# tp7/Sushi

Measured on NVIDIA H100. Metric: subtitle_events_per_s, higher is better.
Workload: dtype f32

## Files before the change

sushi_b200/csrc/sb_fused2.cu:

```cuda
#include "sb_internal.h"
#include <cmath>
#include <cstdlib>
#include <vector>

#include "sb_fused_common.cuh"
#include "sb_fft_smem.cuh"

using namespace sb;
using namespace sbf;

#ifndef SB_V2_SPECIAL_PREFETCH
#define SB_V2_SPECIAL_PREFETCH 1
#endif

namespace {

constexpr int QB = 16384;
constexpr int QT = 512;
constexpr int QNW = QT / 32;
constexpr int Q4 = QB / 4;
constexpr int QBLK = 256;
constexpr int QROW = kQuadRowF2 / 2;
__host__ __device__ constexpr int qa(int i) { return i < Q4 ? (i >> 8) * (2 * QBLK) + (i & (QBLK - 1)) : 2 * Q4; }
__host__ __device__ constexpr int qm(int i) { return i < Q4 ? qa(i) + QBLK : 2 * Q4 + 1; }
static_assert(QROW >= 2 * Q4 + 2 && (QROW * 16) % 128 == 0, "row layout");
constexpr int kDA = 529, kDB = 33;
constexpr int QPHYS = 16 * kDA;
constexpr int kUU = kDA;

struct PackedTables {
    const float2* wb;
    const float4* d1;
    const float4* d2;
};

__device__ constexpr float kC64[8] = {1.0f, 0.99518472667219689f, 0.98078528040323043f, 0.95694033573220882f,
                                      0.92387953251128674f, 0.88192126434835503f, 0.83146961230254524f, 0.77301045336273696f};
__device__ constexpr float kS64[8] = {0.0f, 0.098017140329560602f, 0.19509032201612825f, 0.29028467725446233f,
                                      0.38268343236508978f, 0.47139673682599764f, 0.55557023301960218f, 0.63439328416364549f};

struct C2 { float2 r, i; };
template <bool V> struct BoolTag { static constexpr bool value = V; };

__device__ __forceinline__ float2 neg2(float2 a) { return make_float2(-a.x, -a.y); }
__device__ __forceinline__ float2 add2(float2 a, float2 b) { return make_float2(__fadd_rn(a.x, b.x), __fadd_rn(a.y, b.y)); }
__device__ __forceinline__ float2 sub2(float2 a, float2 b) { return add2(a, neg2(b)); }
__device__ __forceinline__ float2 mul2(float2 a, float2 b) { return make_float2(__fmul_rn(a.x, b.x), __fmul_rn(a.y, b.y)); }
__device__ __forceinline__ float2 fma2(float2 a, float2 b, float2 c) { return make_float2(__fmaf_rn(a.x, b.x, c.x), __fmaf_rn(a.y, b.y, c.y)); }
__device__ __forceinline__ float2 bc(float s) { return make_float2(s, s); }

__device__ __forceinline__ C2 cadd2(C2 a, C2 b) { return {add2(a.r, b.r), add2(a.i, b.i)}; }
__device__ __forceinline__ C2 csub2(C2 a, C2 b) { return {sub2(a.r, b.r), sub2(a.i, b.i)}; }
__device__ __forceinline__ C2 cmul_s(C2 a, float c, float s) {
    C2 o;
    o.r = fma2(a.r, bc(c), mul2(a.i, bc(-s)));
    o.i = fma2(a.r, bc(s), mul2(a.i, bc(c)));
    return o;
}
__device__ __forceinline__ C2 from4(float4 v) { return {make_float2(v.x, v.y), make_float2(v.z, v.w)}; }

__device__ __forceinline__ C2 rot32p(C2 d, int q) {
    if (q == 0) return d;
    if (q == 8) return {neg2(d.i), d.r};
    const float h = 0.70710678118654752f;
    if (q == 4) return {mul2(sub2(d.r, d.i), bc(h)), mul2(add2(d.r, d.i), bc(h))};
    if (q == 12) return {mul2(add2(d.r, d.i), bc(-h)), mul2(sub2(d.r, d.i), bc(h))};
    return cmul_s(d, kC32[q], kS32[q]);
}

template <int HI = 8, int LO = 1>
__device__ __forceinline__ void dft16p(C2 (&v)[16]) {
#pragma unroll
    for (int h = HI; h >= LO; h >>= 1) {
#pragma unroll
        for (int g = 0; g < 16; g += 2 * h) {
#pragma unroll
            for (int a = 0; a < h; ++a) {
                const C2 x = v[g + a], y = v[g + a + h];
                v[g + a] = cadd2(x, y);
                v[g + a + h] = rot32p(csub2(x, y), a * (16 / h));
            }
        }
    }
}

__device__ __forceinline__ constexpr int phys(int n) { return (n >> 9) * kDA + ((n >> 5) & 15) * kDB + (n & 31); }
struct Buf {
    float2* r; float2* i;
    __device__ __forceinline__ C2 ld(int p) const { return {r[p], i[p]}; }
    __device__ __forceinline__ void st(int p, C2 v) const { r[p] = v.r; i[p] = v.i; }
};

struct Rows {
    static constexpr int STRIDE = QROW;
    static __device__ __forceinline__ int unit(int tid, int uu) { return (tid >> 8) * (2 * QBLK) + (tid & (QBLK - 1)) + uu * (2 * QT); }
    static constexpr int USTEP = 2 * QT;
    static __device__ __forceinline__ void load(const float4* row, int u, float4& a, float4& m) { a = __ldg(row + u); m = __ldg(row + u + QBLK); }
    static __device__ __forceinline__ void loadp(const float4* row, int u, bool pred, float4& a, float4& m) {
        const float4 zero4 = make_float4(0.f, 0.f, 0.f, 0.f);
        a = pred ? __ldg(row + u) : zero4;  m = pred ? __ldg(row + u + QBLK) : zero4;
    }
    static __device__ __forceinline__ void load_special(const float4* row, float4& a, float4& m) { a = __ldg(row + qa(Q4)); m = __ldg(row + qm(Q4)); }
};

__device__ __forceinline__ void pack_quad(float2 aR, float2 aI, float2 mR, float2 mI, float c, float s,
                                          C2& lo, C2& hi) {
    const float2 eR = add2(aR, mR), eI = sub2(aI, mI);
    const float2 dR = sub2(aR, mR), dI = add2(aI, mI);
    const float2 wR = make_float2(c, -s), wI = make_float2(s, c);
    const float2 oR = fma2(dR, wR, neg2(mul2(dI, wI)));
    const float2 oI = fma2(dR, wI, mul2(dI, wR));
    const float2 zloR = sub2(eR, oI), zloI = add2(eI, oR);
    const float2 zhiR = add2(eR, oI), zhiI = sub2(oR, eI);
    const float c2 = fmaf(c, c, -s * s), s2 = 2.0f * c * s;
    {
        const float ur = zloR.x + zloR.y, ui = zloI.x + zloI.y;
        const float dr = zloR.x - zloR.y, di = zloI.x - zloI.y;
        lo.r = make_float2(ur, dr * c2 - di * s2);  lo.i = make_float2(ui, dr * s2 + di * c2);
    }
    {
        const float ur = zhiR.y + zhiR.x, ui = zhiI.y + zhiI.x;
        const float dr = zhiR.y - zhiR.x, di = zhiI.y - zhiI.x;
        hi.r = make_float2(ur, -(dr * c2) - di * s2);  hi.i = make_float2(ui, dr * s2 - di * c2);
    }
}

constexpr int kRounds = QB / (QT * 8);
constexpr int kLagsPerRound = QT * 8;

struct Smem {
    Buf buf;
    double2* base;
    unsigned char* lo;
    unsigned char* hi;
    unsigned char* end;
    __device__ __forceinline__ explicit Smem(unsigned char* raw) {
        buf.r = reinterpret_cast<float2*>(raw); buf.i = buf.r + QPHYS;
        base = reinterpret_cast<double2*>(raw + (size_t)QPHYS * 16);
        lo = reinterpret_cast<unsigned char*>(base + kRounds * QNW * 2);
        hi = lo + QB + 16;
        end = hi + QB + 48;
    }
};
constexpr int kSmallBytes = 512;
constexpr size_t kSmemCommon = (size_t)QPHYS * 16 + kRounds * QNW * 2 * sizeof(double2) + (QB + 16) + (QB + 48);

struct Item {
    QueryDesc d; int q; int64_t k, j_blk;
    __device__ __forceinline__ Item(const QueryDesc& dd, int qq, int64_t kk) : d(dd), q(qq), k(kk), j_blk(kk * QB) {}
    __device__ __forceinline__ Item(const QueryDesc* desc, const int* item_query, int64_t item_first, int64_t local) {
        q = __ldg(item_query + local);
        d = desc[q];
        k = d.k0 + (item_first + local - d.itemBase);
        j_blk = k * QB;
    }
};

template <bool WARP_BASES = false>
__device__ __forceinline__ void stage_inputs(const Item& it, int tid, const uint8_t* img8, int64_t img_n,
                                             const double2* ipfx, const Smem& sm, unsigned long long* bar) {
    const int64_t hi0 = (it.j_blk + it.d.tlen) & ~(int64_t)15;
    const int64_t limit = (img_n + 16) & ~(int64_t)15;
    if (tid == 0) {
        int64_t lo_bytes = limit - it.j_blk; if (lo_bytes > QB + 16) lo_bytes = QB + 16; if (lo_bytes < 0) lo_bytes = 0;
        int64_t hi_bytes = limit - hi0;      if (hi_bytes > QB + 48) hi_bytes = QB + 48; if (hi_bytes < 0) hi_bytes = 0;
// ... 379 lines not shown
        const float f_w0q = (float)(Wq + 0.25 + (double)oq);
        const float f_A = (float)(Cw + (double)(oq - bi2 * os));
        float cc[8];
#pragma unroll
        for (int e = 0; e < 2; ++e) {
            const C2 E = buf.ld(ech + kDA * (2 * r + e)), O = buf.ld(ech + kDA * (2 * r + e) + 1);
            const float2 xr = fma2(O.r, bc(wc), fma2(O.i, bc(-ws), E.r));
            const float2 xi = fma2(O.r, bc(ws), fma2(O.i, bc(wc), E.i));
            cc[4 * e + 0] = xr.x; cc[4 * e + 1] = xi.x; cc[4 * e + 2] = xr.y; cc[4 * e + 3] = xi.y;
        }
        const float cmax = fmaxf(fmaxf(fmaxf(cc[0], cc[1]), fmaxf(cc[2], cc[3])), fmaxf(fmaxf(cc[4], cc[5]), fmaxf(cc[6], cc[7])));
        const int64_t j0 = jt + 8 * r;
        const bool some = interior || (j0 < jhi && j0 + 8 > jlo);
        const bool inside = interior || (j0 >= jlo && j0 + 8 <= jhi);
        const float lbn = fmaf(cmax, m2s, f_A - f_delta), ubn = lbn + 2.0f * f_delta;
        const float lbv = lbn * rsqrt_fast(f_w0q + kRunQ) * 0.999999f;
        run_lb[r] = !some ? kSent : (lbn >= 0.f ? lbv : -kSent);
        const float ubv = ubn * rsqrt_fast(f_w0q - kRunQ) * 1.000001f;
        if (inside && f_w0q > 4.0f * kRunQ && ubn >= 0.f) tmin = fminf(tmin, ubv);
        oq += tq[r]; os += ts[r];
    }
#pragma unroll
    for (int o = 16; o > 0; o >>= 1) tmin = fminf(tmin, __shfl_xor_sync(0xffffffffu, tmin, o));
    if (lane == 0) s_min[warp] = tmin;
    fence_proxy_async();
    csync<ID>();
    static_assert(NW == 16, "block minimum over 16 warps");
    float bmin = s_min[lane & (NW - 1)];
#pragma unroll
    for (int o = NW / 2; o > 0; o >>= 1) bmin = fminf(bmin, __shfl_xor_sync(0xffffffffu, bmin, o));
    const float thr = bmin + m_rt;
    const bool all = curve_out != nullptr || !(bmin < sat);
    unsigned left = 0;
#pragma unroll
    for (int r = 0; r < RUNS; ++r) left |= (run_lb[r] <= thr || (all && run_lb[r] < kSent)) ? (1u << r) : 0u;
    if (left && sink.recs != nullptr && !all) {
#pragma unroll 1
        for (int r = 0; r < RUNS; ++r) {
            if (!((left >> r) & 1u)) continue;
            const int slot = atomicAdd(sink.s_cnt, 1);
            if (slot >= kRunSlots) break;
            float cc[8];
            const int k3 = warp;
#pragma unroll
            for (int e = 0; e < 2; ++e) {
                const C2 E = buf.ld(ech + kDA * (2 * r + e)), O = buf.ld(ech + kDA * (2 * r + e) + 1);
                const float2 w = make_float2(kC32[k3], kS32[k3]);
                const float2 xr = fma2(O.r, bc(w.x), fma2(O.i, bc(-w.y), E.r));
                const float2 xi = fma2(O.r, bc(w.y), fma2(O.i, bc(w.x), E.i));
                cc[4 * e + 0] = xr.x; cc[4 * e + 1] = xi.x; cc[4 * e + 2] = xr.y; cc[4 * e + 3] = xi.y;
            }
            float4* r4 = reinterpret_cast<float4*>(sink.recs + slot);
            const int64_t j0 = jt + 8 * r;
            *reinterpret_cast<int4*>(r4) = make_int4(it.q, 1, (int)(unsigned)(j0 & 0xffffffffll), (int)(j0 >> 32));
            r4[1] = make_float4(cc[0], cc[1], cc[2], cc[3]);
            r4[2] = make_float4(cc[4], cc[5], cc[6], cc[7]);
            left &= ~(1u << r);
        }
    }
    unsigned long long best = ~0ull;
    if (__any_sync(0xffffffffu, left != 0u)) {
        unsigned cand = 0;
#pragma unroll 1
        for (int r = 0; r < RUNS; ++r) {
            const bool sel = (left >> r) & 1u;
            if (!__any_sync(0xffffffffu, sel)) continue;
            const int64_t j0 = jt + 8 * r;
            float cc[8];
#pragma unroll
            for (int e = 0; e < 2; ++e) {
                const C2 E = buf.ld(ech + kDA * (2 * r + e)), O = buf.ld(ech + kDA * (2 * r + e) + 1);
                const float2 xr = fma2(O.r, bc(wc), fma2(O.i, bc(-ws), E.r));
                const float2 xi = fma2(O.r, bc(ws), fma2(O.i, bc(wc), E.i));
                cc[4 * e + 0] = xr.x; cc[4 * e + 1] = xi.x; cc[4 * e + 2] = xr.y; cc[4 * e + 3] = xi.y;
            }
            const unsigned long long lo8 = *reinterpret_cast<const unsigned long long*>(sm.lo + 32 * tid + 8 * r);
            const int hb = (int)((j_blk + n) & 15) + 32 * tid + 8 * r;
            const unsigned long long h0 = *reinterpret_cast<const unsigned long long*>(sm.hi + (hb & ~7));
            const unsigned long long h1 = *reinterpret_cast<const unsigned long long*>(sm.hi + (hb & ~7) + 8);
            const unsigned shb = (unsigned)(hb & 7) * 8u;
            const unsigned long long hi8 = shb ? ((h0 >> shb) | (h1 << (64u - shb))) : h0;
            const int2 off = s_w0[r * QT + tid];
            const float f_w0q = (float)(Wq + 0.25 + (double)off.y);
            const float f_A = (float)(Cw + (double)(off.y - bi2 * off.x));
            float v8[8];
            float vmin = kSent;
            int rq = 0, rs = 0;
#pragma unroll
            for (int i = 0; i < 8; ++i) {
                const float frq = (float)rq;
                const float num = fmaf(cc[i], m2s, fmaf(m2b, (float)rs, f_A + frq));
                const float v = num * rsqrt_fast(f_w0q + frq);
                const bool valid = sel && j0 + i >= jlo && j0 + i < jhi;
                v8[i] = valid ? v : kSent;
                vmin = fminf(vmin, v8[i]);
                const int lo = (int)((lo8 >> (8 * i)) & 0xffu), hi = (int)((hi8 >> (8 * i)) & 0xffu);
                const int dd = hi - lo;
                rq += (hi + lo) * dd; rs += dd;
            }
#pragma unroll
            for (int o = 16; o > 0; o >>= 1) vmin = fminf(vmin, __shfl_xor_sync(0xffffffffu, vmin, o));
            const float thrw = fminf(thr, vmin + m_rt);
#pragma unroll
            for (int i = 0; i < 8; ++i) cand |= (v8[i] < kSent && (v8[i] <= thrw || all)) ? (1u << (r * 8 + i)) : 0u;
        }
        while (cand) {
            const int bit = __ffs((int)cand) - 1;
            cand &= cand - 1;
            const int r = bit >> 3, i = bit & 7;
            const int m = 32 * tid + bit;
            const int64_t j = j_blk + m;
            const int jj = m >> 2;
            const int ca = (jj & 15) * kDA + ((jj >> 4) & 15) * kDB + 2 * (jj >> 8);
            const C2 E = buf.ld(ca), O = buf.ld(ca + 1);
            const float2 w = make_float2(kC32[jj >> 8], kS32[jj >> 8]);
            const bool second = (m & 2) != 0;
            const float er = second ? E.r.y : E.r.x, ei = second ? E.i.y : E.i.x, orr = second ? O.r.y : O.r.x, oi = second ? O.i.y : O.i.x;
            const float xr = fmaf(orr, w.x, fmaf(oi, -w.y, er)), xi = fmaf(orr, w.y, fmaf(oi, w.x, ei));
            const double cc = (double)((m & 1) ? xi : xr) * scale;
            const unsigned long long lo8 = *reinterpret_cast<const unsigned long long*>(sm.lo + 32 * tid + 8 * r);
            const int hb = (int)((j_blk + n) & 15) + 32 * tid + 8 * r;
            const unsigned long long h0 = *reinterpret_cast<const unsigned long long*>(sm.hi + (hb & ~7));
            const unsigned long long h1 = *reinterpret_cast<const unsigned long long*>(sm.hi + (hb & ~7) + 8);
            const unsigned shb = (unsigned)(hb & 7) * 8u;
            const unsigned long long hi8 = shb ? ((h0 >> shb) | (h1 << (64u - shb))) : h0;
            const unsigned long long keep = i ? (~0ull >> (8 * (8 - i))) : 0ull;
            const unsigned la = (unsigned)(lo8 & keep), lb = (unsigned)((lo8 & keep) >> 32), ha = (unsigned)(hi8 & keep), hb2 = (unsigned)((hi8 & keep) >> 32);
            const int rq = (int)__dp4a(ha, ha, __dp4a(hb2, hb2, 0u)) - (int)__dp4a(la, la, __dp4a(lb, lb, 0u));
            const int rs = (int)__dp4a(ha, 0x01010101u, __dp4a(hb2, 0x01010101u, 0u)) - (int)__dp4a(la, 0x01010101u, __dp4a(lb, 0x01010101u, 0u));
            const int2 off = s_w0[r * QT + tid];
            const double wsum = (Ws + (double)off.x) + (double)rs, wsq = (Wq + (double)off.y) + (double)rq;
            const float v = sqdiff_exact(cc, wsum, wsq, a, b, tsum, tsq, n_ab);
            if (curve_out) curve_out[d.curveOff + (j - jlo)] = v;
            const unsigned long long key = ((unsigned long long)__float_as_uint(v) << 32) | (unsigned int)(j - jlo);
            best = key < best ? key : best;
        }
        if (best != ~0ull) atomicMin(keys + it.q, best);
    }
    fence_proxy_async();
    csync<ID>();
    after_read();
}

template <typename S> struct QueryStreams { const float4* Xhat; int64_t nblk; const S* img; int64_t img_n; const double2* ipfx; const double2* tpfx; };
template <typename S>
__device__ __forceinline__ QueryStreams<S> select_streams(const StreamEntry* streams, const int2* slots, int q) {
    const int2 sl = slots[q];
    const StreamEntry si = streams[sl.x];
    return {reinterpret_cast<const float4*>(si.specq), si.nblk, static_cast<const S*>(si.raw), si.n, si.pfx, streams[sl.y].pfx};
}
#define SB_SELECT_STREAMS(q) do { const QueryStreams<S> qs__ = select_streams<S>(streams, slots, (q)); \
    Xhat = qs__.Xhat; nblk = qs__.nblk; img = qs__.img; img_n = qs__.img_n; ipfx = qs__.ipfx; tpfx = qs__.tpfx; } while (0)

template <typename S, int EPI, bool MULTI = false>
__global__ void __launch_bounds__(QT, 1)
k_match_packed(const float4* __restrict__ That, int64_t part_first,
               const float4* __restrict__ Xhat, int64_t nblk,
               const S* __restrict__ img, int64_t img_n,
               const double2* __restrict__ ipfx, const double2* __restrict__ tpfx,
               const QueryDesc* __restrict__ desc, const int* __restrict__ item_query, int64_t item_first,
               PackedTables tab, unsigned long long* __restrict__ keys, float* __restrict__ curve_out,
               RunRecord* __restrict__ recs, int* __restrict__ rec_count,
               const StreamEntry* __restrict__ streams = nullptr, const int2* __restrict__ slots = nullptr) {
    constexpr int T = QT, NW = QNW;
    constexpr bool is_u8 = sizeof(S) == 1;
    extern __shared__ __align__(16) unsigned char smem_raw[];
    const Smem sm(smem_raw);
    unsigned long long* s_bar = reinterpret_cast<unsigned long long*>(sm.end);
    unsigned long long* s_best = s_bar + 1;
    float* s_min = reinterpret_cast<float*>(s_best + NW);
    int* s_cnt = reinterpret_cast<int*>(sm.end + kRunCountOff());
    const RunSink sink = {EPI == 3 && recs ? recs + (size_t)blockIdx.x * kRunSlots : nullptr, s_cnt};
    float4* s_sp = reinterpret_cast<float4*>(sm.end + kSmallBytes);
    int2* s_w0 = EPI >= 2 && is_u8 ? reinterpret_cast<int2*>(sm.end + kSmallBytes + kSpecialBytes) : nullptr;
    const Buf& buf = sm.buf;

    const int tid = threadIdx.x, lane = tid & 31, warp = tid >> 5;
    const Item it(desc, item_query, item_first, blockIdx.x);
    const QueryDesc& d = it.d;
    if constexpr (MULTI) SB_SELECT_STREAMS(it.q);

    if (is_u8) {
        if (tid == 0) mbar_init(s_bar, 1);
        stage_inputs<EPI == 3>(it, tid, reinterpret_cast<const uint8_t*>(img), img_n, ipfx, sm, s_bar);
    }
    if (EPI == 3 && tid == 96) *s_cnt = 0;
    if (EPI >= 2 && tid == 64) query_constants<S>(reinterpret_cast<double2*>(sm.end + kQueryConstOff()), d, img_n, ipfx, tpfx);

    {
        int P = d.P;
        if (it.k + P > nblk) P = (int)(nblk - it.k);
        typedef Rows R;
        const float4* tp = That + (d.partBase - part_first) * (int64_t)R::STRIDE;
        const float4* xp = Xhat + it.k * (int64_t)R::STRIDE;
        const float2 wbase = __ldg(tab.wb + tid);
        const int tm = (T - tid) & (T - 1);
        const int col = phys(tid), mcol = phys(tm);
        const bool sp_pref = EPI >= 2 && SB_V2_SPECIAL_PREFETCH && special_fits(d.P, 1);
        if (sp_pref && warp == NW - 1) special_prefetch(s_sp, tp, xp, d.P, 1, it.k, nblk, lane);
        constexpr int U = 4;
#pragma unroll 1
        for (int half = 0; half < 2; ++half) {
            const int i0 = R::unit(tid, half * U);
            QuadAcc acc[U];
#pragma unroll
            for (int u = 0; u < U; ++u) acc[u].zero();
#pragma unroll 1
            for (int p = 0; p < P; ++p) {
                const float4* t = tp + (int64_t)p * R::STRIDE;
                const float4* x = xp + (int64_t)p * R::STRIDE;
                float4 ta[U], tmm[U], xa[U], xm[U];
#pragma unroll
                for (int u = 0; u < U; ++u) {
                    R::load(t, i0 + u * R::USTEP, ta[u], tmm[u]);
                    R::load(x, i0 + u * R::USTEP, xa[u], xm[u]);
                }
#pragma unroll
                for (int u = 0; u < U; ++u) acc[u].mac(ta[u], tmm[u], xa[u], xm[u]);
            }
#pragma unroll
            for (int u = 0; u < U; ++u) {
                const int uu = half * U + u;
                const float c = wbase.x * kC64[uu] - wbase.y * kS64[uu];
                const float s = wbase.x * kS64[uu] + wbase.y * kC64[uu];
                C2 lo, hi;
                pack_quad(acc[u].aR, acc[u].aI, acc[u].mR, acc[u].mI, c, s, lo, hi);
                buf.st(col + kUU * uu, lo);
                if (tid != 0) buf.st(mcol + kUU * (15 - uu), hi);
                else if (uu != 0) buf.st(mcol + kUU * (16 - uu), hi);
            }
        }
        if (warp == NW - 1) {
            if (sp_pref) {
                cp_async_commit_wait_all();
                __syncwarp();
                const C2 lo = special_from_smem(s_sp, d.P, 0, lane);
                if (lane == 0) buf.st(phys(Q4), lo);
            } else {
                const C2 lo = special_quad(tp, xp, P, lane);
                if (lane == 0) buf.st(phys(Q4), lo);
            }
        }
    }
    csync<0>();

    fft_passes_dif<0>(buf, tid, tab, is_u8);
    if constexpr (EPI == 3) finish_item_v3<0>(it, tid, sm, s_bar, 0u, s_min, s_w0, img_n, keys, curve_out, [] {}, sink);
    else finish_item<S, 0>(it, tid, sm, s_bar, 0u, s_best, s_min, img, img_n, ipfx, tpfx, keys, curve_out, [] {});
    if (EPI == 3 && rec_count && tid == 0) rec_count[blockIdx.x] = *s_cnt < kRunSlots ? *s_cnt : kRunSlots;
}

constexpr int kParkF4 = 16 * QT;

__device__ __forceinline__ void unpark(const float4* pk, const Buf& buf, int col, int mcol, int tid) {
#pragma unroll
    for (int uu = 0; uu < 8; ++uu) {
        const C2 lo = from4(park_ld(pk + (2 * uu) * QT)), hi = from4(park_ld(pk + (2 * uu + 1) * QT));
        buf.st(col + kUU * uu, lo);
        if (tid != 0) buf.st(mcol + kUU * (15 - uu), hi);
        else if (uu != 0) buf.st(mcol + kUU * (16 - uu), hi);
    }
}

template <typename S, int EPI, bool MULTI = false>
__global__ void __launch_bounds__(QT, 1)
k_match_pair(const float4* __restrict__ That, int64_t part_first,
             const float4* __restrict__ Xhat, int64_t nblk,
             const S* __restrict__ img, int64_t img_n,
             const double2* __restrict__ ipfx, const double2* __restrict__ tpfx,
             const QueryDesc* __restrict__ desc, const int* __restrict__ pair_query, int64_t pair_first, int64_t n_pairs,
             float4* __restrict__ park, int* __restrict__ park_busy, int park_slots,
             PackedTables tab, unsigned long long* __restrict__ keys, float* __restrict__ curve_out,
             RunRecord* __restrict__ recs, int* __restrict__ rec_count,
             const StreamEntry* __restrict__ streams = nullptr, const int2* __restrict__ slots = nullptr) {
    constexpr int T = QT, NW = QNW;
    constexpr bool is_u8 = sizeof(S) == 1;
    extern __shared__ __align__(16) unsigned char smem_raw[];
    const Smem sm(smem_raw);
    unsigned long long* s_bar = reinterpret_cast<unsigned long long*>(sm.end);
    unsigned long long* s_best = s_bar + 1;
    float* s_min = reinterpret_cast<float*>(s_best + NW);
    int* s_slot = reinterpret_cast<int*>(s_min + NW);
    int* s_cnt = reinterpret_cast<int*>(sm.end + kRunCountOff());
    int* s_next_q = reinterpret_cast<int*>(sm.end + kNextOff());
    QueryDesc* s_next_d = reinterpret_cast<QueryDesc*>(sm.end + kNextOff() + 16);
    float4* s_sp = reinterpret_cast<float4*>(sm.end + kSmallBytes);
    int2* s_w0 = EPI >= 2 && is_u8 ? reinterpret_cast<int2*>(sm.end + kSmallBytes + kSpecialBytes) : nullptr;
    const Buf& buf = sm.buf;

    const int tid = threadIdx.x, lane = tid & 31, warp = tid >> 5;
    if (tid == 64) *s_slot = park_acquire(park_busy, park_slots, (int)(blockIdx.x % (unsigned)park_slots));
    if (is_u8 && tid == 0) mbar_init(s_bar, 1);
    if (EPI == 3 && tid == 32) *s_cnt = 0;
    csync<0>();
    float4* const pk = park + (size_t)*s_slot * kParkF4 + tid;
    const int tm = (T - tid) & (T - 1);
    const int col = phys(tid), mcol = phys(tm);
    const float2 wbase = __ldg(tab.wb + tid);
    unsigned phase = 0;

    constexpr bool kPersistent = EPI == 3, kPrefetch = kPersistent;
    int64_t pi = blockIdx.x;
    do {
    const bool first = !kPrefetch || pi == (int64_t)blockIdx.x;
    const int q = first ? __ldg(pair_query + pi) : *s_next_q;
    const QueryDesc d = first ? desc[q] : *s_next_d;
    if constexpr (MULTI) SB_SELECT_STREAMS(q);
    const int64_t pi_next = pi + gridDim.x;
    int q_next = 0;
    if (kPrefetch && tid == 32 && pi_next < n_pairs) q_next = __ldg(pair_query + pi_next);
    const int lp = (int)(pair_first + pi - d.groupBase);
    const bool has2 = 2 * lp + 1 < d.nk;
    const Item it0(d, q, d.k0 + 2 * lp), it1(d, q, d.k0 + 2 * lp + 1);
    const RunSink sink = {EPI == 3 && recs ? recs + (size_t)pi * kRunSlots : nullptr, s_cnt};

    if (is_u8) stage_inputs<EPI == 3>(it0, tid, reinterpret_cast<const uint8_t*>(img), img_n, ipfx, sm, s_bar);
    if (EPI >= 2 && tid == 64) query_constants<S>(reinterpret_cast<double2*>(sm.end + kQueryConstOff()), d, img_n, ipfx, tpfx);
    C2 sp1 = {make_float2(0.f, 0.f), make_float2(0.f, 0.f)};
    {
        typedef Rows R;
        const int64_t k = it0.k;
        const float4* tp = That + (d.partBase - part_first) * (int64_t)R::STRIDE;
        const float4* xp = Xhat + k * (int64_t)R::STRIDE;
        const bool sp_pref = EPI >= 2 && SB_V2_SPECIAL_PREFETCH && special_fits(d.P, 2);
        if (sp_pref && warp == NW - 1) special_prefetch(s_sp, tp, xp, d.P, 2, k, nblk, lane);
        constexpr int U = 2;
#pragma unroll 1
        for (int grp = 0; grp < 8 / U; ++grp) {
            const int i0 = R::unit(tid, grp * U);
            QuadAcc a0[U], a1[U];
            float4 xa[U], xm[U];
#pragma unroll
            for (int u = 0; u < U; ++u) {
                a0[u].zero(); a1[u].zero();
                R::load(xp, i0 + u * R::USTEP, xa[u], xm[u]);
            }
#pragma unroll 2
            for (int p = 0; p < d.P; ++p) {
                const float4* t = tp + (int64_t)p * R::STRIDE;
                const float4* x = xp + (int64_t)(p + 1) * R::STRIDE;
                const bool next_row = k + p + 1 < nblk;
                float4 ta[U], tmm[U], xna[U], xnm[U];
#pragma unroll
                for (int u = 0; u < U; ++u) {
                    R::load(t, i0 + u * R::USTEP, ta[u], tmm[u]);
                    R::loadp(x, i0 + u * R::USTEP, next_row, xna[u], xnm[u]);
                }
#pragma unroll
                for (int u = 0; u < U; ++u) {
                    a0[u].mac(ta[u], tmm[u], xa[u], xm[u]);
                    a1[u].mac(ta[u], tmm[u], xna[u], xnm[u]);
                    xa[u] = xna[u]; xm[u] = xnm[u];
                }
            }
#pragma unroll
            for (int u = 0; u < U; ++u) {
                const int uu = grp * U + u;
                const float c = wbase.x * kC64[uu] - wbase.y * kS64[uu];
                const float s = wbase.x * kS64[uu] + wbase.y * kC64[uu];
                C2 lo, hi;
                pack_quad(a0[u].aR, a0[u].aI, a0[u].mR, a0[u].mI, c, s, lo, hi);
                buf.st(col + kUU * uu, lo);
                if (tid != 0) buf.st(mcol + kUU * (15 - uu), hi);
                else if (uu != 0) buf.st(mcol + kUU * (16 - uu), hi);
                pack_quad(a1[u].aR, a1[u].aI, a1[u].mR, a1[u].mI, c, s, lo, hi);
                park_st(pk + (2 * uu) * QT, make_float4(lo.r.x, lo.r.y, lo.i.x, lo.i.y));
                park_st(pk + (2 * uu + 1) * QT, make_float4(hi.r.x, hi.r.y, hi.i.x, hi.i.y));
            }
        }
        if (warp == NW - 1) {
            if (sp_pref) {
                cp_async_commit_wait_all();
                __syncwarp();
                const C2 lo = special_from_smem(s_sp, d.P, 0, lane);
                if (lane == 0) buf.st(phys(Q4), lo);
                if (has2) sp1 = special_from_smem(s_sp, d.P, 1, lane);
            } else {
                int P0 = d.P; if (k + P0 > nblk) P0 = (int)(nblk - k);
                const C2 lo = special_quad(tp, xp, P0, lane);
                if (lane == 0) buf.st(phys(Q4), lo);
                if (has2) {
                    int P1 = d.P; if (k + 1 + P1 > nblk) P1 = (int)(nblk - k - 1);
                    sp1 = special_quad(tp, xp + R::STRIDE, P1, lane);
                }
            }
        }
    }
    csync<0>();
    if (kPrefetch && tid == 32 && pi_next < n_pairs) {
        *s_next_q = q_next;
        const float4* src = reinterpret_cast<const float4*>(desc + q_next);
        static_assert(sizeof(QueryDesc) == 80, "five 16-byte copies");
#pragma unroll
        for (int k = 0; k < 5; ++k) cp_async16(reinterpret_cast<float4*>(s_next_d) + k, src + k);
    }

    fft_passes_dif<0>(buf, tid, tab, true);
    auto stage_second = [&] { if (is_u8 && has2) stage_inputs<EPI == 3>(it1, tid, reinterpret_cast<const uint8_t*>(img), img_n, ipfx, sm, s_bar); };
    if constexpr (EPI == 3) finish_item_v3<0>(it0, tid, sm, s_bar, phase & 1u, s_min, s_w0, img_n, keys, curve_out, stage_second, sink);
    else finish_item<S, 0>(it0, tid, sm, s_bar, phase & 1u, s_best, s_min, img, img_n, ipfx, tpfx, keys, curve_out, stage_second);
    ++phase;

    if (has2) {
        unpark(pk, buf, col, mcol, tid);
        if (tid == (NW - 1) * 32) buf.st(phys(Q4), sp1);
        csync<0>();
        fft_passes_dif<0>(buf, tid, tab, is_u8);
        if constexpr (EPI == 3) finish_item_v3<0>(it1, tid, sm, s_bar, phase & 1u, s_min, s_w0, img_n, keys, curve_out, [] {}, sink);
        else finish_item<S, 0>(it1, tid, sm, s_bar, phase & 1u, s_best, s_min, img, img_n, ipfx, tpfx, keys, curve_out, [] {});
        ++phase;
    }
    if (EPI == 3 && rec_count && tid == 32) { rec_count[pi] = *s_cnt < kRunSlots ? *s_cnt : kRunSlots; *s_cnt = 0; }
    } while (kPersistent && (pi += gridDim.x) < n_pairs);
    csync<0>();
    if (tid == 64) park_release(park_busy + *s_slot);
}

template <typename S, bool MULTI = false>
__global__ void __launch_bounds__(128)
k_finish_runs(const RunRecord* __restrict__ recs, const int* __restrict__ rec_count, int64_t n_ctas,
              const QueryDesc* __restrict__ desc, const double2* __restrict__ ipfx, int64_t img_n,
              const double2* __restrict__ tpfx, unsigned long long* __restrict__ keys,
              const StreamEntry* __restrict__ streams = nullptr, const int2* __restrict__ slots = nullptr) {
    const int64_t idx = (int64_t)blockIdx.x * blockDim.x + threadIdx.x;
    const int64_t cta = idx / kRunSlots;
    const int slot = (int)(idx - cta * kRunSlots);
    if (cta >= n_ctas || slot >= rec_count[cta]) return;
    const float4* r4 = reinterpret_cast<const float4*>(recs + cta * kRunSlots + slot);
    const int4 head = *reinterpret_cast<const int4*>(r4);
    const float4 c0 = r4[1], c1 = r4[2];
    const float cc[8] = {c0.x, c0.y, c0.z, c0.w, c1.x, c1.y, c1.z, c1.w};
    const int q = head.x;
    const int64_t j0 = (int64_t)(unsigned)head.z | ((int64_t)head.w << 32);
    if constexpr (MULTI) {
        const int2 sl = slots[q];
        ipfx = streams[sl.x].pfx; img_n = streams[sl.x].n; tpfx = streams[sl.y].pfx;
    }
    const QueryDesc d = desc[q];
    const int64_t n = d.tlen, jlo = d.lag0, jhi = d.lag0 + d.nlags;
    const double2 t_hi = tpfx[d.toff + n], t_lo = tpfx[d.toff];
    const double tsum = t_hi.x - t_lo.x, tsq = t_hi.y - t_lo.y;
    const double a = (double)Acc<S>::centre(ipfx[img_n].x, (double)img_n);
    const double b = (double)Acc<S>::centre(tsum, (double)n);
    const double n_ab = (double)n * a * b;
    const double scale = 1.0 / (double)(2 * QB);
    unsigned long long best = ~0ull;
#pragma unroll 1
    for (int i = 0; i < 8; ++i) {
        const int64_t j = j0 + i;
        if (j < jlo || j >= jhi) continue;
        const double2 p_hi = ipfx[j + n], p_lo = ipfx[j];
        const float v = sqdiff_exact((double)cc[i] * scale, p_hi.x - p_lo.x, p_hi.y - p_lo.y, a, b, tsum, tsq, n_ab);
        const unsigned long long key = ((unsigned long long)__float_as_uint(v) << 32) | (unsigned int)(j - jlo);
        best = key < best ? key : best;
    }
    if (best != ~0ull) atomicMin(keys + q, best);
}

__global__ void k_fill_pair_query(const QueryDesc* __restrict__ desc, int q_begin, int64_t pair_first, int* __restrict__ pair_query, int group) {
    const int q = q_begin + blockIdx.x;
    const int64_t base = desc[q].groupBase - pair_first;
    const int np = (desc[q].nk + group - 1) / group;
    for (int i = threadIdx.x; i < np; i += blockDim.x) pair_query[base + i] = q;
}

template <typename S, int MODE, bool MULTI = false>
__global__ void __launch_bounds__(Cfg<14>::T, 1)
k_forward_quad(const S* __restrict__ src, int64_t src_n, const double2* __restrict__ pfx,
               const QueryDesc* __restrict__ desc, int q_begin, int q_end, int64_t row_first,
               FusedTables tab, float4* __restrict__ out,
               const StreamEntry* __restrict__ streams = nullptr, const int2* __restrict__ slots = nullptr,
               const int2* __restrict__ row_list = nullptr, int64_t rows = -1) {
    typedef Cfg<14> C;
    constexpr int N = C::N, T = C::T, B = C::N;
    constexpr int NT2 = C::R2 * 32, NT3 = C::R3 * 32;
    extern __shared__ __align__(16) unsigned char smem_raw[];
    float2* buf = reinterpret_cast<float2*>(smem_raw);
    float2* s_t2 = buf + pad(N) + 1;
    float2* s_a3 = s_t2 + NT2;
    float2* s_b3 = s_a3 + NT3;
    int* s_q = reinterpret_cast<int*>(s_b3 + NT3);
    const int tid = threadIdx.x;
    for (int i = tid; i < NT2; i += T) s_t2[i] = __ldg(tab.t2 + i);
    for (int i = tid; i < NT3; i += T) { s_a3[i] = __ldg(tab.a3 + i); s_b3[i] = __ldg(tab.b3 + i); }

    for (int64_t item = blockIdx.x; rows < 0 ? item == blockIdx.x : item < rows; item += gridDim.x) {
        const S* xs = src;
        const double2* xpfx = pfx;
        float4* xout = out;
        int64_t off, len;
        float centre;
        int64_t row = row_first + item, out_row = item;
        if constexpr (MULTI && MODE == 0) {
            const int2 rl = row_list[item];
            const StreamEntry se = streams[rl.x];
            xs = static_cast<const S*>(se.raw); xpfx = se.pfx;
            xout = reinterpret_cast<float4*>(se.specq);
            row = out_row = rl.y;
            off = row * B;
            len = se.n - off; if (len > 2 * B) len = 2 * B; if (len < 0) len = 0;
            centre = Acc<S>::centre(xpfx[se.n].x, (double)se.n);
        } else if (MODE == 0) {
            off = row * B;
            len = src_n - off; if (len > 2 * B) len = 2 * B; if (len < 0) len = 0;
            centre = Acc<S>::centre(pfx[src_n].x, (double)src_n);
        } else {
            int lo = q_begin, n = q_end - q_begin;
            while (n > 1) {
                const int s = (n + T - 1) / T, m = (n + s - 1) / s;
                auto le = [&](int t) { return t == 0 || (t < m && desc[lo + t * s].partBase <= row); };
                if (le(tid) && !le(tid + 1)) *s_q = tid;
                __syncthreads();
                const int c = *s_q;
                __syncthreads();
                lo += c * s;
                n = c == m - 1 ? n - c * s : s;
            }
            const int q = lo;
            const QueryDesc d = desc[q];
            if constexpr (MULTI) { xs = static_cast<const S*>(streams[slots[q].y].raw); xpfx = streams[slots[q].y].pfx; }
            const int64_t seg0 = (row - d.partBase) * B;
            off = d.toff + seg0;
            len = d.tlen - seg0; if (len > B) len = B;
            centre = Acc<S>::centre(xpfx[d.toff + d.tlen].x - xpfx[d.toff].x, (double)d.tlen);
        }
        const S* x = xs + off;
#pragma unroll
        for (int k = 0; k < B / T; ++k) {
            const int n = tid + k * T;
            const int64_t i0 = 2 * (int64_t)n;
            const float a = i0 < len ? (float)x[i0] - centre : 0.f;
            const float b = i0 + 1 < len ? (float)x[i0 + 1] - centre : 0.f;
            buf[pad(n)] = make_float2(a, -b);
        }
        __syncthreads();
        ifft_smem<C::R3, false>(buf, s_t2, s_a3, s_b3);
        auto bins = [&](int k, float2& xk, float2& xbk) {
            const float2 zk = buf[pad(k)];
            const float2 zp = buf[pad(k == 0 ? 0 : B - k)];
            const float2 A = make_float2(zk.x, -zk.y), P = make_float2(zp.x, zp.y);
            const float2 xe = make_float2(0.5f * (A.x + P.x), 0.5f * (A.y + P.y));
            const float2 dd = make_float2(A.x - P.x, A.y - P.y);
            const float2 xo = make_float2(0.5f * dd.y, -0.5f * dd.x);
            const float2 w = __ldg(tab.w + k);
            const float2 tv = cmul(make_float2(w.x, -w.y), xo);
            xk = make_float2(xe.x + tv.x, xe.y + tv.y);
            xbk = make_float2(xe.x - tv.x, -(xe.y - tv.y));
        };
        float4* o = xout + out_row * QROW;
        for (int i = tid; i <= Q4; i += T) {
            float2 x_i, x_bi, x_h, x_hb;
            bins(i, x_i, x_bi);
            bins(B / 2 - i, x_h, x_hb);
            o[qa(i)] = make_float4(x_i.x, x_hb.x, x_i.y, x_hb.y);
            o[qm(i)] = make_float4(x_bi.x, x_h.x, x_bi.y, x_h.y);
        }
        __syncthreads();
    }
}

size_t forward_smem_bytes14() {
    typedef Cfg<14> C;
    return ((size_t)(C::N + (C::N >> 5) + 1) + C::R2 * 32 + 2 * C::R3 * 32) * sizeof(float2) + 64;
}

static_assert(8 + QNW * 8 + QNW * 4 + 4 <= kRunCountOff() && kRunCountOff() + 4 <= kNextOff() &&
              kNextOff() + 16 + (int)sizeof(QueryDesc) <= kQueryConstOff() && kQueryConstOff() + 32 <= kSmallBytes, "small shared-memory area");
size_t packed_smem_bytes(int epi = 1) {
    return epi >= 2 ? kSmemCommon + kSmallBytes + kSpecialBytes + (size_t)kRounds * QT * sizeof(int2)
                    : kSmemCommon + kSmallBytes;
}

constexpr int kPackedTableCount = 3;
std::vector<float> packed_table_values(size_t (&off)[kPackedTableCount]) {
    const double pi = 3.14159265358979323846;
    const size_t nb = 512 * 2, nd1 = 8 * 512 * 4, nd2 = 8 * 32 * 4;
    off[0] = 0; off[1] = nb; off[2] = nb + nd1;
    std::vector<float> h(off[2] + nd2);
    auto pairs = [&](size_t at, int K, double N) {
        for (int a = 0; a < 8; ++a)
            for (int k = 0; k < K; ++k)
                for (int e = 0; e < 2; ++e) {
                    const double ang = 2.0 * pi * (double)((2 * a + e) * k) / N;
                    h[at + ((size_t)a * K + k) * 4 + 2 * e] = (float)cos(ang); h[at + ((size_t)a * K + k) * 4 + 2 * e + 1] = (float)sin(ang);
                }
    };
    for (int t = 0; t < 512; ++t) { h[off[0] + 2 * t] = (float)cos(pi * t / QB); h[off[0] + 2 * t + 1] = (float)sin(pi * t / QB); }
    pairs(off[1], 512, 8192.0);
    pairs(off[2], 32, 512.0);
    return h;
}

PackedTables packed_tables_at(const float* base, const size_t (&off)[kPackedTableCount]) {
    PackedTables t;
    t.wb = reinterpret_cast<const float2*>(base + off[0]);
    t.d1 = reinterpret_cast<const float4*>(base + off[1]);
    t.d2 = reinterpret_cast<const float4*>(base + off[2]);
    return t;
}

#ifndef SB_EMULATE
float* g_ptab_dev = nullptr;
PackedTables g_ptab;

int ensure_packed_tables(PackedTables* out) {
    if (!g_ptab_dev) {
        size_t off[kPackedTableCount];
        const std::vector<float> h = packed_table_values(off);
        SB_CUDA(cudaMalloc(&g_ptab_dev, h.size() * sizeof(float)));
        SB_CUDA(cudaMemcpy(g_ptab_dev, h.data(), h.size() * sizeof(float), cudaMemcpyHostToDevice));
        g_ptab = packed_tables_at(g_ptab_dev, off);
    }
    *out = g_ptab;
    return SB_OK;
}

__global__ void k_fill_item_query2(const QueryDesc* __restrict__ desc, int q_begin, int64_t item_first,
                                   int* __restrict__ item_query) {
    const int q = q_begin + blockIdx.x;
    const int64_t base = desc[q].itemBase - item_first;
    const int nk = desc[q].nk;
    for (int i = threadIdx.x; i < nk; i += blockDim.x) item_query[base + i] = q;
}

int* g_item_query2 = nullptr;
int64_t g_item_query2_cap = 0;

template <typename S, int MODE, bool MULTI = false>
int launch_forward_quad_typed(const sb_stream* src, const QueryDesc* d_desc, int q_begin, int q_end,
                              int64_t row_first, int64_t rows, float2* out, const MultiArgs* m = nullptr,
                              const int2* row_list = nullptr) {
    Ctx& c = ctx();
    FusedTables tab;
    SB_TRY(fused_tables(&tab));
    static bool attr_set = false;
    const size_t smem = forward_smem_bytes14();
    if (!attr_set) {
        SB_CUDA(cudaFuncSetAttribute(k_forward_quad<S, MODE, MULTI>, cudaFuncAttributeMaxDynamicSharedMemorySize, (int)smem));
        attr_set = true;
    }
    const int64_t grid = std::min<int64_t>(rows, c.sm_count);
    k_forward_quad<S, MODE, MULTI><<<(unsigned)grid, Cfg<14>::T, smem, c.stream>>>(
        static_cast<const S*>(src->d_raw), src->n, src->d_pfx, d_desc, q_begin, q_end, row_first, tab,
        reinterpret_cast<float4*>(out), MULTI ? m->d_streams : nullptr, MULTI ? m->d_slots : nullptr, row_list, rows);
    SB_CUDA(cudaGetLastError());
    return SB_OK;
}

int ensure_item_query(int64_t n) {
    if (g_item_query2_cap < n) {
        cudaStreamSynchronize(ctx().stream);
        cudaFree(g_item_query2); g_item_query2 = nullptr; g_item_query2_cap = 0;
        SB_CUDA(cudaMalloc(&g_item_query2, sizeof(int) * (size_t)n));
        g_item_query2_cap = n;
    }
    return SB_OK;
}

RunRecord* g_run_recs = nullptr;
int* g_run_count = nullptr;
int64_t g_run_cap = 0;
constexpr int64_t kRunChunk = 1 << 19;

int ensure_run_records(int64_t n_ctas) {
    if (g_run_cap < n_ctas) {
        cudaStreamSynchronize(ctx().stream);
        cudaFree(g_run_recs); cudaFree(g_run_count); g_run_recs = nullptr; g_run_count = nullptr; g_run_cap = 0;
        SB_CUDA(cudaMalloc(&g_run_recs, sizeof(RunRecord) * (size_t)n_ctas * kRunSlots));
        SB_CUDA(cudaMalloc(&g_run_count, sizeof(int) * (size_t)n_ctas));
        g_run_cap = n_ctas;
    }
    return SB_OK;
}

float4* g_park = nullptr;
int* g_park_busy = nullptr;
int g_park_slots = 0;

int ensure_park() {
    Ctx& c = ctx();
    if (g_park_slots != c.sm_count) {
        cudaStreamSynchronize(c.stream);
        cudaFree(g_park); cudaFree(g_park_busy); g_park = nullptr; g_park_busy = nullptr; g_park_slots = 0;
        SB_CUDA(cudaMalloc(&g_park, sizeof(float4) * kParkF4 * (size_t)c.sm_count));
        SB_CUDA(cudaMalloc(&g_park_busy, sizeof(int) * (size_t)c.sm_count));
        SB_CUDA(cudaMemsetAsync(g_park_busy, 0, sizeof(int) * (size_t)c.sm_count, c.stream));
        g_park_slots = c.sm_count;
    }
    return SB_OK;
}

const sb_stream kNoStream{};

template <typename S, bool MULTI>
int launch_finish_runs(const sb_stream* image, const sb_stream* tmpl, const QueryDesc* d_desc, int64_t n_ctas, unsigned long long* d_keys,
                       const MultiArgs* m) {
    Ctx& c = ctx();
    const int64_t threads = n_ctas * kRunSlots;
    k_finish_runs<S, MULTI><<<(unsigned)((threads + 127) / 128), 128, 0, c.stream>>>(g_run_recs, g_run_count, n_ctas, d_desc, image->d_pfx, image->n,
                                                                                   tmpl->d_pfx, d_keys, MULTI ? m->d_streams : nullptr,
                                                                                   MULTI ? m->d_slots : nullptr);
    c.launches += 1;
    SB_CUDA(cudaGetLastError());
    return SB_OK;
}

template <typename S, int EPI, bool MULTI>
int launch_packed_typed(const sb_stream* image, const sb_stream* tmpl, const float2* d_parts, int64_t part_first,
                        const QueryDesc* d_desc, int64_t item_first, int64_t n_items, const PackedTables& tab,
                        unsigned long long* d_keys, float* d_curve, const MultiArgs* m) {
    Ctx& c = ctx();
    static bool attr_set = false;
    const size_t smem = packed_smem_bytes(EPI);
    if (!attr_set) {
        SB_CUDA(cudaFuncSetAttribute(k_match_packed<S, EPI, MULTI>, cudaFuncAttributeMaxDynamicSharedMemorySize, (int)smem));
        attr_set = true;
    }
    const bool records = EPI == 3 && d_curve == nullptr;
    const int64_t max_grid = records ? kRunChunk : (int64_t)1 << 30;
    for (int64_t i0 = 0; i0 < n_items; i0 += max_grid) {
        const int64_t ni = std::min<int64_t>(max_grid, n_items - i0);
        if (records) SB_TRY(ensure_run_records(ni));
        k_match_packed<S, EPI, MULTI><<<(unsigned)ni, QT, smem, c.stream>>>(
            reinterpret_cast<const float4*>(d_parts), part_first, reinterpret_cast<const float4*>(image->d_specq), image->nblkq,
            static_cast<const S*>(image->d_raw), image->n, image->d_pfx, tmpl->d_pfx, d_desc, g_item_query2 + i0, item_first + i0,
            tab, d_keys, d_curve, records ? g_run_recs : nullptr, records ? g_run_count : nullptr,
            MULTI ? m->d_streams : nullptr, MULTI ? m->d_slots : nullptr);
        if (records) SB_TRY((launch_finish_runs<S, MULTI>(image, tmpl, d_desc, ni, d_keys, m)));
    }
    SB_CUDA(cudaGetLastError());
    return SB_OK;
}

template <typename S, int EPI, bool MULTI>
int launch_pair_typed(const sb_stream* image, const sb_stream* tmpl, const float2* d_parts, int64_t part_first,
                      const QueryDesc* d_desc, int64_t pair_first, int64_t n_pairs, const PackedTables& tab,
                      unsigned long long* d_keys, float* d_curve, const MultiArgs* m) {
    Ctx& c = ctx();
    static bool attr_set = false;
    const size_t smem = packed_smem_bytes(EPI) + 16;
    if (!attr_set) {
        SB_CUDA(cudaFuncSetAttribute(k_match_pair<S, EPI, MULTI>, cudaFuncAttributeMaxDynamicSharedMemorySize, (int)smem));
        attr_set = true;
    }
    const bool records = EPI == 3 && d_curve == nullptr;
    const int64_t max_grid = records ? kRunChunk : (int64_t)1 << 30;
    for (int64_t i0 = 0; i0 < n_pairs; i0 += max_grid) {
        const int64_t ni = std::min<int64_t>(max_grid, n_pairs - i0);
        if (records) SB_TRY(ensure_run_records(ni));
        const int64_t grid = EPI == 3 ? std::min<int64_t>(ni, c.sm_count) : ni;
        k_match_pair<S, EPI, MULTI><<<(unsigned)grid, QT, smem, c.stream>>>(
            reinterpret_cast<const float4*>(d_parts), part_first, reinterpret_cast<const float4*>(image->d_specq), image->nblkq,
            static_cast<const S*>(image->d_raw), image->n, image->d_pfx, tmpl->d_pfx, d_desc, g_item_query2 + i0, pair_first + i0, ni,
            g_park, g_park_busy, g_park_slots, tab, d_keys, d_curve, records ? g_run_recs : nullptr, records ? g_run_count : nullptr,
            MULTI ? m->d_streams : nullptr, MULTI ? m->d_slots : nullptr);
        SB_CUDA(cudaGetLastError());
        if (records) SB_TRY((launch_finish_runs<S, MULTI>(image, tmpl, d_desc, ni, d_keys, m)));
    }
    return SB_OK;
}

#define SB_DISPATCH_MATCH1(FN, M, dtype, ...) \
    ((dtype) != SB_U8        ? FN<float, 1, M>(__VA_ARGS__) \
     : ctx().epilogue == 3   ? FN<uint8_t, 3, M>(__VA_ARGS__) : FN<uint8_t, 1, M>(__VA_ARGS__))
#define SB_DISPATCH_MATCH(FN, image, tmpl, multi, ...) \
    ((multi) ? SB_DISPATCH_MATCH1(FN, true, (multi)->dtype, &kNoStream, &kNoStream, __VA_ARGS__, multi) \
             : SB_DISPATCH_MATCH1(FN, false, (image)->dtype, image, tmpl, __VA_ARGS__, multi))

}

namespace sb {

int launch_match_packed(const sb_stream* image, const sb_stream* tmpl, const float2* d_parts, int64_t part_first,
                        const QueryDesc* d_desc, int q_begin, int q_end, int64_t item_first, int64_t n_items,
                        unsigned long long* d_keys, float* d_curve, const MultiArgs* multi) {
    Ctx& c = ctx();
    PackedTables tab;
    SB_TRY(ensure_packed_tables(&tab));
    SB_TRY(ensure_item_query(n_items));
    k_fill_item_query2<<<(unsigned)(q_end - q_begin), 128, 0, c.stream>>>(d_desc, q_begin, item_first, g_item_query2);
    c.launches += 1;
    return SB_DISPATCH_MATCH(launch_packed_typed, image, tmpl, multi, d_parts, part_first, d_desc, item_first, n_items, tab, d_keys, d_curve);
}

int launch_match_pair(const sb_stream* image, const sb_stream* tmpl, const float2* d_parts, int64_t part_first,
                      const QueryDesc* d_desc, int q_begin, int q_end, int64_t pair_first, int64_t n_pairs,
                      unsigned long long* d_keys, float* d_curve, const MultiArgs* multi) {
    Ctx& c = ctx();
    PackedTables tab;
    SB_TRY(ensure_packed_tables(&tab));
    SB_TRY(ensure_item_query(n_pairs));
    SB_TRY(ensure_park());
    k_fill_pair_query<<<(unsigned)(q_end - q_begin), 128, 0, c.stream>>>(d_desc, q_begin, pair_first, g_item_query2, 2);
    c.launches += 1;
    return SB_DISPATCH_MATCH(launch_pair_typed, image, tmpl, multi, d_parts, part_first, d_desc, pair_first, n_pairs, tab, d_keys, d_curve);
}

int launch_block_spectra_quad(const sb_stream* s, int64_t k_first, int64_t rows, float2* out) {
    return s->dtype == SB_U8 ? launch_forward_quad_typed<uint8_t, 0>(s, nullptr, 0, 0, k_first, rows, out)
                             : launch_forward_quad_typed<float, 0>(s, nullptr, 0, 0, k_first, rows, out);
}

int launch_block_spectra_quad_multi(const MultiArgs& m, const int2* d_row_list, int64_t n_rows) {
    return m.dtype == SB_U8 ? launch_forward_quad_typed<uint8_t, 0, true>(&kNoStream, nullptr, 0, 0, 0, n_rows, nullptr, &m, d_row_list)
                            : launch_forward_quad_typed<float, 0, true>(&kNoStream, nullptr, 0, 0, 0, n_rows, nullptr, &m, d_row_list);
}

int launch_part_spectra_quad(const sb_stream* tmpl, const QueryDesc* d_desc, int q_begin, int q_end,
                             int64_t part_first, int64_t rows, float2* out, const MultiArgs* multi) {
    if (multi)
        return multi->dtype == SB_U8 ? launch_forward_quad_typed<uint8_t, 1, true>(&kNoStream, d_desc, q_begin, q_end, part_first, rows, out, multi)
                                     : launch_forward_quad_typed<float, 1, true>(&kNoStream, d_desc, q_begin, q_end, part_first, rows, out, multi);
    return tmpl->dtype == SB_U8 ? launch_forward_quad_typed<uint8_t, 1>(tmpl, d_desc, q_begin, q_end, part_first, rows, out)
                                : launch_forward_quad_typed<float, 1>(tmpl, d_desc, q_begin, q_end, part_first, rows, out);
}

void packed_release_tables() {
    if (g_ptab_dev) cudaFree(g_ptab_dev);
    g_ptab_dev = nullptr;
    cudaFree(g_item_query2); g_item_query2 = nullptr; g_item_query2_cap = 0;
    cudaFree(g_run_recs); cudaFree(g_run_count); g_run_recs = nullptr; g_run_count = nullptr; g_run_cap = 0;
    cudaFree(g_park); cudaFree(g_park_busy); g_park = nullptr; g_park_busy = nullptr; g_park_slots = 0;
}

}
#else
}
#endif
```

Before: 49000.

## Process groups of consecutive items per CTA in packed match kernel

The packed matching kernel now has each CTA loop over up to four consecutive work items when the EPI==3 epilogue is used. It reuses barrier initialisation and skips per-query setup (stream selection, query constants) when the next item belongs to the same query. The goal is to amortise CTA launch and setup costs across items, at the cost of fewer CTAs and items within a CTA running serially. A compile-time SB_MATCH_PHASE probe mode is also added; it defaults to off.

```diff
diff --git a/sushi_b200/csrc/sb_fused2.cu b/sushi_b200/csrc/sb_fused2.cu
--- a/sushi_b200/csrc/sb_fused2.cu
+++ b/sushi_b200/csrc/sb_fused2.cu
@@ -11,6 +11,9 @@
 
 #ifndef SB_V2_SPECIAL_PREFETCH
 #define SB_V2_SPECIAL_PREFETCH 1
+#endif
+#ifndef SB_MATCH_PHASE
+#define SB_MATCH_PHASE 0
 #endif
 
 namespace {
@@ -696,7 +699,10 @@
 #define SB_SELECT_STREAMS(q) do { const QueryStreams<S> qs__ = select_streams<S>(streams, slots, (q)); \
     Xhat = qs__.Xhat; nblk = qs__.nblk; img = qs__.img; img_n = qs__.img_n; ipfx = qs__.ipfx; tpfx = qs__.tpfx; } while (0)
 
-template <typename S, int EPI, bool MULTI = false>
+constexpr int kPackedGroup = 4;
+template <int EPI> constexpr int packed_group() { return EPI == 3 ? kPackedGroup : 1; }
+
+template <typename S, int EPI, bool MULTI = false, int G = 1>
 __global__ void __launch_bounds__(QT, 1)
 k_match_packed(const float4* __restrict__ That, int64_t part_first,
                const float4* __restrict__ Xhat, int64_t nblk,
@@ -705,7 +711,8 @@
                const QueryDesc* __restrict__ desc, const int* __restrict__ item_query, int64_t item_first,
                PackedTables tab, unsigned long long* __restrict__ keys, float* __restrict__ curve_out,
                RunRecord* __restrict__ recs, int* __restrict__ rec_count,
-               const StreamEntry* __restrict__ streams = nullptr, const int2* __restrict__ slots = nullptr) {
+               const StreamEntry* __restrict__ streams = nullptr, const int2* __restrict__ slots = nullptr,
+               int64_t n_items = 0) {
     constexpr int T = QT, NW = QNW;
     constexpr bool is_u8 = sizeof(S) == 1;
     extern __shared__ __align__(16) unsigned char smem_raw[];
@@ -714,24 +721,29 @@
     unsigned long long* s_best = s_bar + 1;
     float* s_min = reinterpret_cast<float*>(s_best + NW);
     int* s_cnt = reinterpret_cast<int*>(sm.end + kRunCountOff());
-    const RunSink sink = {EPI == 3 && recs ? recs + (size_t)blockIdx.x * kRunSlots : nullptr, s_cnt};
     float4* s_sp = reinterpret_cast<float4*>(sm.end + kSmallBytes);
     int2* s_w0 = EPI >= 2 && is_u8 ? reinterpret_cast<int2*>(sm.end + kSmallBytes + kSpecialBytes) : nullptr;
     const Buf& buf = sm.buf;
 
     const int tid = threadIdx.x, lane = tid & 31, warp = tid >> 5;
-    const Item it(desc, item_query, item_first, blockIdx.x);
+    const int64_t i_end = (int64_t)blockIdx.x * G + G < n_items ? (int64_t)blockIdx.x * G + G : n_items;
+    int64_t local = (int64_t)blockIdx.x * G;
+    int q = __ldg(item_query + local);
+    int64_t k = -1;
+    if (is_u8 && tid == 0) mbar_init(s_bar, 1);
+    if (EPI == 3 && tid == 0) *s_cnt = 0;
+    unsigned phase = 0;
+    for (;;) {
+    const bool new_query = k < 0;
+    const Item it(desc[q], q, new_query ? desc[q].k0 + (item_first + local - desc[q].itemBase) : k);
     const QueryDesc& d = it.d;
-    if constexpr (MULTI) SB_SELECT_STREAMS(it.q);
-
-    if (is_u8) {
-        if (tid == 0) mbar_init(s_bar, 1);
-        stage_inputs<EPI == 3>(it, tid, reinterpret_cast<const uint8_t*>(img), img_n, ipfx, sm, s_bar);
-    }
-    if (EPI == 3 && tid == 96) *s_cnt = 0;
-    if (EPI >= 2 && tid == 64) query_constants<S>(reinterpret_cast<double2*>(sm.end + kQueryConstOff()), d, img_n, ipfx, tpfx);
-
-    {
+    if constexpr (MULTI) { if (new_query) SB_SELECT_STREAMS(it.q); }
+    const RunSink sink = {EPI == 3 && recs ? recs + (size_t)local * kRunSlots : nullptr, s_cnt};
+
+    if (is_u8) stage_inputs<EPI == 3>(it, tid, reinterpret_cast<const uint8_t*>(img), img_n, ipfx, sm, s_bar);
+    if (EPI >= 2 && tid == 64 && new_query) query_constants<S>(reinterpret_cast<double2*>(sm.end + kQueryConstOff()), d, img_n, ipfx, tpfx);
+
+    if (SB_MATCH_PHASE != 2) {
         int P = d.P;
         if (it.k + P > nblk) P = (int)(nblk - it.k);
         typedef Rows R;
@@ -787,11 +799,25 @@
         }
     }
     csync<0>();
+    if constexpr (SB_MATCH_PHASE == 1) {
+        if (is_u8) { mbar_wait(s_bar, phase & 1u); cp_async_commit_wait_all(); }
+        if (tid == 0) {
+            atomicMin(keys + it.q, (unsigned long long)((__float_as_uint(buf.r[0].x) ^ __float_as_uint(buf.i[QPHYS - 1].y)) & 0x3fffffffu) << 32);
+            if (EPI == 3 && rec_count) rec_count[local] = 0;
+        }
+        csync<0>();
+    } else {
 
     fft_passes_dif<0>(buf, tid, tab, is_u8);
-    if constexpr (EPI == 3) finish_item_v3<0>(it, tid, sm, s_bar, 0u, s_min, s_w0, img_n, keys, curve_out, [] {}, sink);
-    else finish_item<S, 0>(it, tid, sm, s_bar, 0u, s_best, s_min, img, img_n, ipfx, tpfx, keys, curve_out, [] {});
-    if (EPI == 3 && rec_count && tid == 0) rec_count[blockIdx.x] = *s_cnt < kRunSlots ? *s_cnt : kRunSlots;
+    if constexpr (EPI == 3) finish_item_v3<0>(it, tid, sm, s_bar, phase & 1u, s_min, s_w0, img_n, keys, curve_out, [] {}, sink);
+    else finish_item<S, 0>(it, tid, sm, s_bar, phase & 1u, s_best, s_min, img, img_n, ipfx, tpfx, keys, curve_out, [] {});
+    if (EPI == 3 && tid == 0) { if (rec_count) rec_count[local] = *s_cnt < kRunSlots ? *s_cnt : kRunSlots; *s_cnt = 0; }
+    }
+    ++phase;
+    if (G == 1 || ++local >= i_end) break;
+    k = it.k + 1;
+    if (k >= (int64_t)d.k0 + d.nk) { q = __ldg(item_query + local); k = -1; }
+    }
 }
 
 constexpr int kParkF4 = 16 * QT;
@@ -962,15 +988,15 @@
 
 template <typename S, bool MULTI = false>
 __global__ void __launch_bounds__(128)
-k_finish_runs(const RunRecord* __restrict__ recs, const int* __restrict__ rec_count, int64_t n_ctas,
+k_finish_runs(const RunRecord* __restrict__ recs, const int* __restrict__ rec_count, int64_t n_groups,
               const QueryDesc* __restrict__ desc, const double2* __restrict__ ipfx, int64_t img_n,
               const double2* __restrict__ tpfx, unsigned long long* __restrict__ keys,
               const StreamEntry* __restrict__ streams = nullptr, const int2* __restrict__ slots = nullptr) {
     const int64_t idx = (int64_t)blockIdx.x * blockDim.x + threadIdx.x;
-    const int64_t cta = idx / kRunSlots;
-    const int slot = (int)(idx - cta * kRunSlots);
-    if (cta >= n_ctas || slot >= rec_count[cta]) return;
-    const float4* r4 = reinterpret_cast<const float4*>(recs + cta * kRunSlots + slot);
+    const int64_t g = idx / kRunSlots;
+    const int slot = (int)(idx - g * kRunSlots);
+    if (g >= n_groups || slot >= rec_count[g]) return;
+    const float4* r4 = reinterpret_cast<const float4*>(recs + g * kRunSlots + slot);
     const int4 head = *reinterpret_cast<const int4*>(r4);
     const float4 c0 = r4[1], c1 = r4[2];
     const float cc[8] = {c0.x, c0.y, c0.z, c0.w, c1.x, c1.y, c1.z, c1.w};
@@ -1206,13 +1232,13 @@
 int64_t g_run_cap = 0;
 constexpr int64_t kRunChunk = 1 << 19;
 
-int ensure_run_records(int64_t n_ctas) {
-    if (g_run_cap < n_ctas) {
+int ensure_run_records(int64_t n_groups) {
+    if (g_run_cap < n_groups) {
         cudaStreamSynchronize(ctx().stream);
         cudaFree(g_run_recs); cudaFree(g_run_count); g_run_recs = nullptr; g_run_count = nullptr; g_run_cap = 0;
-        SB_CUDA(cudaMalloc(&g_run_recs, sizeof(RunRecord) * (size_t)n_ctas * kRunSlots));
-        SB_CUDA(cudaMalloc(&g_run_count, sizeof(int) * (size_t)n_ctas));
-        g_run_cap = n_ctas;
+        SB_CUDA(cudaMalloc(&g_run_recs, sizeof(RunRecord) * (size_t)n_groups * kRunSlots));
+        SB_CUDA(cudaMalloc(&g_run_count, sizeof(int) * (size_t)n_groups));
+        g_run_cap = n_groups;
     }
     return SB_OK;
 }
@@ -1237,11 +1263,11 @@
 const sb_stream kNoStream{};
 
 template <typename S, bool MULTI>
-int launch_finish_runs(const sb_stream* image, const sb_stream* tmpl, const QueryDesc* d_desc, int64_t n_ctas, unsigned long long* d_keys,
+int launch_finish_runs(const sb_stream* image, const sb_stream* tmpl, const QueryDesc* d_desc, int64_t n_groups, unsigned long long* d_keys,
                        const MultiArgs* m) {
     Ctx& c = ctx();
-    const int64_t threads = n_ctas * kRunSlots;
-    k_finish_runs<S, MULTI><<<(unsigned)((threads + 127) / 128), 128, 0, c.stream>>>(g_run_recs, g_run_count, n_ctas, d_desc, image->d_pfx, image->n,
+    const int64_t threads = n_groups * kRunSlots;
+    k_finish_runs<S, MULTI><<<(unsigned)((threads + 127) / 128), 128, 0, c.stream>>>(g_run_recs, g_run_count, n_groups, d_desc, image->d_pfx, image->n,
                                                                                    tmpl->d_pfx, d_keys, MULTI ? m->d_streams : nullptr,
                                                                                    MULTI ? m->d_slots : nullptr);
     c.launches += 1;
@@ -1257,7 +1283,7 @@
     static bool attr_set = false;
     const size_t smem = packed_smem_bytes(EPI);
     if (!attr_set) {
-        SB_CUDA(cudaFuncSetAttribute(k_match_packed<S, EPI, MULTI>, cudaFuncAttributeMaxDynamicSharedMemorySize, (int)smem));
+        SB_CUDA(cudaFuncSetAttribute(k_match_packed<S, EPI, MULTI, packed_group<EPI>()>, cudaFuncAttributeMaxDynamicSharedMemorySize, (int)smem));
         attr_set = true;
     }
     const bool records = EPI == 3 && d_curve == nullptr;
@@ -1265,11 +1291,12 @@
     for (int64_t i0 = 0; i0 < n_items; i0 += max_grid) {
         const int64_t ni = std::min<int64_t>(max_grid, n_items - i0);
         if (records) SB_TRY(ensure_run_records(ni));
-        k_match_packed<S, EPI, MULTI><<<(unsigned)ni, QT, smem, c.stream>>>(
+        constexpr int G = packed_group<EPI>();
+        k_match_packed<S, EPI, MULTI, G><<<(unsigned)((ni + G - 1) / G), QT, smem, c.stream>>>(
             reinterpret_cast<const float4*>(d_parts), part_first, reinterpret_cast<const float4*>(image->d_specq), image->nblkq,
             static_cast<const S*>(image->d_raw), image->n, image->d_pfx, tmpl->d_pfx, d_desc, g_item_query2 + i0, item_first + i0,
             tab, d_keys, d_curve, records ? g_run_recs : nullptr, records ? g_run_count : nullptr,
-            MULTI ? m->d_streams : nullptr, MULTI ? m->d_slots : nullptr);
+            MULTI ? m->d_streams : nullptr, MULTI ? m->d_slots : nullptr, ni);
         if (records) SB_TRY((launch_finish_runs<S, MULTI>(image, tmpl, d_desc, ni, d_keys, m)));
     }
     SB_CUDA(cudaGetLastError());
```

Result: no change. 49440 (median of 6 runs) (+0.9%).
